# Eclectic-Sheep/sheeprl

Hardware: NVIDIA H100
Metric: Dreamer-V3 train-steps/sec (S, bs16 seq64 horizon15, 64x64x3 obs) (higher is better)
Workload: dtype f32

## Files before the change

### sheeprl_b200/csrc/gemm_tc.cu

```cuda
#include <cuda.h>
#include <cudaTypedefs.h>

#include <mutex>
#include <unordered_map>

#include "common.cuh"

namespace {

constexpr int BM = 128, BK = 32;
constexpr int NTHREADS = 384;
constexpr int NSPLIT_THREADS = 96;
constexpr int NCONS_WARPS = 8;
constexpr int PRODUCER_REGS = 56, CONSUMER_REGS = 224;
template <int BN> constexpr int stages_for() { return BN == 128 ? 3 : 5; }

__device__ __forceinline__ uint32_t smem_u32(const void* p) { return (uint32_t)__cvta_generic_to_shared(p); }

__device__ __forceinline__ void mbar_init(uint64_t* bar, uint32_t count) {
  asm volatile("mbarrier.init.shared::cta.b64 [%0], %1;" ::"r"(smem_u32(bar)), "r"(count) : "memory");
}
__device__ __forceinline__ void mbar_expect_tx(uint64_t* bar, uint32_t bytes) {
  asm volatile("mbarrier.arrive.expect_tx.shared::cta.b64 _, [%0], %1;" ::"r"(smem_u32(bar)), "r"(bytes) : "memory");
}
__device__ __forceinline__ void mbar_arrive(uint64_t* bar) {
  asm volatile("mbarrier.arrive.shared::cta.b64 _, [%0];" ::"r"(smem_u32(bar)) : "memory");
}
__device__ __forceinline__ bool mbar_try_wait(uint64_t* bar, uint32_t parity) {
  uint32_t ok;
  asm volatile(
      "{\n\t"
      ".reg .pred p;\n\t"
      "mbarrier.try_wait.parity.shared::cta.b64 p, [%1], %2;\n\t"
      "selp.u32 %0, 1, 0, p;\n\t"
      "}"
      : "=r"(ok)
      : "r"(smem_u32(bar)), "r"(parity)
      : "memory");
  return ok != 0;
}
__device__ __forceinline__ void mbar_wait(uint64_t* bar, uint32_t parity) {
  if (mbar_try_wait(bar, parity)) return;
  const long long t0 = clock64();
  while (!mbar_try_wait(bar, parity)) {
    if (clock64() - t0 > 2000000000LL) asm volatile("trap;");
  }
}
__device__ __forceinline__ bool elect_one() {
  uint32_t pred;
  asm volatile(
      "{\n\t"
      ".reg .pred p;\n\t"
      "elect.sync _|p, 0xffffffff;\n\t"
      "selp.u32 %0, 1, 0, p;\n\t"
      "}"
      : "=r"(pred));
  return pred != 0;
}
__device__ __forceinline__ void tma_load_2d(void* smem_dst, const CUtensorMap* map, uint64_t* bar, int c0, int c1) {
  asm volatile(
      "cp.async.bulk.tensor.2d.shared::cluster.global.mbarrier::complete_tx::bytes [%0], [%1, {%3, %4}], [%2];" ::"r"(
          smem_u32(smem_dst)),
      "l"(map), "r"(smem_u32(bar)), "r"(c0), "r"(c1)
      : "memory");
}
__device__ __forceinline__ void tma_load_4d(void* smem_dst, const CUtensorMap* map, uint64_t* bar, int c0, int c1, int c2,
                                            int c3) {
  asm volatile(
      "cp.async.bulk.tensor.4d.shared::cluster.global.mbarrier::complete_tx::bytes [%0], [%1, {%3, %4, %5, %6}], [%2];" ::"r"(
          smem_u32(smem_dst)),
      "l"(map), "r"(smem_u32(bar)), "r"(c0), "r"(c1), "r"(c2), "r"(c3)
      : "memory");
}

__device__ __forceinline__ void wgmma_tf32(float (&d)[32], const uint32_t (&a)[4], uint64_t desc_b, int scale_d) {
  asm volatile(
      "{\n\t.reg .pred p;\n\tsetp.ne.b32 p, %37, 0;\n\twgmma.mma_async.sync.aligned.m64n64k8.f32.tf32.tf32 {%0, %1, %2, %3, %4, %5, %6, %7, %8, %9, %10, %11, %12, %13, %14, %15, %16, %17, %18, %19, %20, %21, %22, %23, %24, %25, %26, %27, %28, %29, %30, %31}, {%32, %33, %34, %35}, %36, p, 1, 1;\n\t}"
      : "+f"(d[0]), "+f"(d[1]), "+f"(d[2]), "+f"(d[3]), "+f"(d[4]), "+f"(d[5]), "+f"(d[6]), "+f"(d[7]), "+f"(d[8]), "+f"(d[9]), "+f"(d[10]), "+f"(d[11]), "+f"(d[12]), "+f"(d[13]), "+f"(d[14]), "+f"(d[15]), "+f"(d[16]), "+f"(d[17]), "+f"(d[18]), "+f"(d[19]), "+f"(d[20]), "+f"(d[21]), "+f"(d[22]), "+f"(d[23]), "+f"(d[24]), "+f"(d[25]), "+f"(d[26]), "+f"(d[27]), "+f"(d[28]), "+f"(d[29]), "+f"(d[30]), "+f"(d[31])
      : "r"(a[0]), "r"(a[1]), "r"(a[2]), "r"(a[3]), "l"(desc_b), "r"(scale_d));
}
__device__ __forceinline__ void wgmma_tf32(float (&d)[64], const uint32_t (&a)[4], uint64_t desc_b, int scale_d) {
  asm volatile(
      "{\n\t.reg .pred p;\n\tsetp.ne.b32 p, %69, 0;\n\twgmma.mma_async.sync.aligned.m64n128k8.f32.tf32.tf32 {%0, %1, %2, %3, %4, %5, %6, %7, %8, %9, %10, %11, %12, %13, %14, %15, %16, %17, %18, %19, %20, %21, %22, %23, %24, %25, %26, %27, %28, %29, %30, %31, %32, %33, %34, %35, %36, %37, %38, %39, %40, %41, %42, %43, %44, %45, %46, %47, %48, %49, %50, %51, %52, %53, %54, %55, %56, %57, %58, %59, %60, %61, %62, %63}, {%64, %65, %66, %67}, %68, p, 1, 1;\n\t}"
      : "+f"(d[0]), "+f"(d[1]), "+f"(d[2]), "+f"(d[3]), "+f"(d[4]), "+f"(d[5]), "+f"(d[6]), "+f"(d[7]), "+f"(d[8]), "+f"(d[9]), "+f"(d[10]), "+f"(d[11]), "+f"(d[12]), "+f"(d[13]), "+f"(d[14]), "+f"(d[15]), "+f"(d[16]), "+f"(d[17]), "+f"(d[18]), "+f"(d[19]), "+f"(d[20]), "+f"(d[21]), "+f"(d[22]), "+f"(d[23]), "+f"(d[24]), "+f"(d[25]), "+f"(d[26]), "+f"(d[27]), "+f"(d[28]), "+f"(d[29]), "+f"(d[30]), "+f"(d[31]), "+f"(d[32]), "+f"(d[33]), "+f"(d[34]), "+f"(d[35]), "+f"(d[36]), "+f"(d[37]), "+f"(d[38]), "+f"(d[39]), "+f"(d[40]), "+f"(d[41]), "+f"(d[42]), "+f"(d[43]), "+f"(d[44]), "+f"(d[45]), "+f"(d[46]), "+f"(d[47]), "+f"(d[48]), "+f"(d[49]), "+f"(d[50]), "+f"(d[51]), "+f"(d[52]), "+f"(d[53]), "+f"(d[54]), "+f"(d[55]), "+f"(d[56]), "+f"(d[57]), "+f"(d[58]), "+f"(d[59]), "+f"(d[60]), "+f"(d[61]), "+f"(d[62]), "+f"(d[63])
      : "r"(a[0]), "r"(a[1]), "r"(a[2]), "r"(a[3]), "l"(desc_b), "r"(scale_d));
}
__device__ __forceinline__ void wgmma_fence() { asm volatile("wgmma.fence.sync.aligned;" ::: "memory"); }
__device__ __forceinline__ void wgmma_commit() { asm volatile("wgmma.commit_group.sync.aligned;" ::: "memory"); }
__device__ __forceinline__ void wgmma_wait_all() { asm volatile("wgmma.wait_group.sync.aligned 0;" ::: "memory"); }
template <int N>
__device__ __forceinline__ void fence_regs(float (&r)[N]) {
#pragma unroll
  for (int i = 0; i < N; ++i) asm volatile("" : "+f"(r[i])::"memory");
}
template <int N, int W>
__device__ __forceinline__ void fence_regs(uint32_t (&r)[N][W]) {
#pragma unroll
  for (int i = 0; i < N; ++i)
#pragma unroll
    for (int j = 0; j < W; ++j) asm volatile("" : "+r"(r[i][j])::"memory");
}

__device__ __forceinline__ uint64_t make_desc(uint32_t smem_addr) {
  uint64_t d = 0;
  d |= (uint64_t)((smem_addr & 0x3FFFF) >> 4);
  d |= (uint64_t)1 << 16;
  d |= (uint64_t)(1024 >> 4) << 32;
  d |= (uint64_t)1 << 62;
  return d;
}

__device__ __forceinline__ uint32_t kmajor_off(int r, int k) {
  return (uint32_t)(r * 128 + ((((k >> 2) ^ r) & 7) << 4) + (k & 3) * 4);
}
__device__ __forceinline__ uint32_t mnmajor_off(int r, int k) {
  return (uint32_t)((r >> 5) * 4096 + k * 128 + (((((r & 31) >> 2) ^ k) & 7) << 4) + (r & 3) * 4);
}

template <int BN>
struct Smem {
  static constexpr int STAGES = stages_for<BN>();
  float a[STAGES][BM * BK];
  float b[STAGES][BN * BK];
  float b_hi[STAGES][BN * BK];
  float b_lo[STAGES][BN * BK];
  uint64_t full[STAGES], split[STAGES], empty[STAGES];
};

constexpr int CH = 4;

constexpr int MODE_GEMM = 0, MODE_DOWN = 1, MODE_UP = 2;
constexpr int MODE_UP4 = 3;
constexpr int GROUP_M = 16;
struct TileGeo {
  int mode;
  int h, w, NB;
  int bw, bh, bn;
  int tiles_x, tiles_y;
  int chunks;
  int Cout;
  int ksplits;
  float* part;
  int mpad, ldw;
  int force_part;
  int passes;
  int a_mn, b_mn;
  int mtiles;
  int ntiles;
  int wg;
};

template <int BN, int PASSES>
__global__ void __launch_bounds__(NTHREADS, 1)
gemm_tc_kernel(const __grid_constant__ CUtensorMap mapA, const __grid_constant__ CUtensorMap mapB, float* __restrict__ C,
               const float* __restrict__ bias, int M, int N, int K, int ldc, int accumulate, const TileGeo geo) {
  constexpr int STAGES = Smem<BN>::STAGES;
  extern __shared__ __align__(1024) unsigned char smem_raw[];
  Smem<BN>& s = *reinterpret_cast<Smem<BN>*>((reinterpret_cast<uintptr_t>(smem_raw) + 1023) & ~(uintptr_t)1023);
  const int warp = threadIdx.x >> 5, lane = threadIdx.x & 31;
  const int mtiles = geo.mtiles * geo.ntiles, tstride = gridDim.y;
  auto tile_mn = [&](int id, int& tm, int& tn) {
    if (geo.ntiles == 1) { tm = id; tn = 0; return; }
    const int per = GROUP_M * geo.ntiles, grp = id / per, first = grp * GROUP_M;
    const int gsz = min(GROUP_M, geo.mtiles - first), r = id - grp * per;
    tn = r / gsz;
    tm = first + (r - tn * gsz);
  };
  int kb_base = 0, nkb = (K + BK - 1) / BK;
  if (geo.mode == MODE_GEMM && geo.ksplits > 1) {
    const int per = (nkb + geo.ksplits - 1) / geo.ksplits;
    kb_base = (int)blockIdx.z * per;
    nkb = min(per, nkb - kb_base);
  }
  const int py = (int)blockIdx.z >> 1, px = (int)blockIdx.z & 1;
  auto tile_origin = [&](int id, int& tx0, int& ty0, int& tn0) {
    tx0 = (id % geo.tiles_x) * geo.bw;
    ty0 = ((id / geo.tiles_x) % geo.tiles_y) * geo.bh;
    tn0 = (id / (geo.tiles_x * geo.tiles_y)) * geo.bn;
  };

  if (threadIdx.x == 0) {
    for (int i = 0; i < STAGES; ++i) {
      mbar_init(&s.full[i], 1);
      mbar_init(&s.split[i], NSPLIT_THREADS / 32);
      mbar_init(&s.empty[i], NCONS_WARPS);
    }
    asm volatile("fence.mbarrier_init.release.cluster;" ::: "memory");
  }
  __syncthreads();

  if (warp < 4) {
    asm volatile("setmaxnreg.dec.sync.aligned.u32 %0;" ::"n"(PRODUCER_REGS));
    if (warp == 0) {
      const bool leader = elect_one();
      int it = 0;
      for (int tile = blockIdx.y; tile < mtiles; tile += tstride) {
        int tm, tn;
        tile_mn(tile, tm, tn);
        const int m0 = tm * BM, n0 = tn * BN;
        int tx0 = 0, ty0 = 0, tn0 = 0;
        if (geo.mode != MODE_GEMM) tile_origin(tm, tx0, ty0, tn0);
        for (int kb = 0; kb < nkb; ++kb, ++it) {
          const int st = it % STAGES;
          if (it >= STAGES) mbar_wait(&s.empty[st], ((it / STAGES) - 1) & 1);
          if (leader) {
            mbar_expect_tx(&s.full[st], (uint32_t)((BM + BN) * BK * sizeof(float)));
            if (geo.mode == MODE_GEMM) {
              const int k0 = (kb_base + kb) * BK;
              if (geo.wg) {
                const int x0 = k0 % geo.w, y0 = (k0 / geo.w) % geo.h, i0 = k0 / (geo.w * geo.h);
                for (int j = 0; j < BM / 32; ++j) {
                  const int r0 = m0 + 32 * j, tap = r0 / geo.Cout, ch = r0 - tap * geo.Cout;
                  tma_load_4d(s.a[st] + j * 1024, &mapA, &s.full[st], ch, 2 * x0 - 1 + (tap & 3), 2 * y0 - 1 + (tap >> 2), i0);
                }
              } else if (!geo.a_mn) tma_load_2d(s.a[st], &mapA, &s.full[st], k0, m0);
              else
                for (int j = 0; j < BM / 32; ++j) tma_load_2d(s.a[st] + j * 1024, &mapA, &s.full[st], m0 + 32 * j, k0);
              if (!geo.b_mn) tma_load_2d(s.b[st], &mapB, &s.full[st], k0, n0);
              else
                for (int j = 0; j < BN / 32; ++j) tma_load_2d(s.b[st] + j * 1024, &mapB, &s.full[st], n0 + 32 * j, k0);
            } else {
              const int tap = kb / geo.chunks, ch = (kb - tap * geo.chunks) * BK;
              int x, y;
              if (geo.mode == MODE_DOWN)     { x = 2 * tx0 - 1 + (tap & 3); y = 2 * ty0 - 1 + (tap >> 2); }
              else if (geo.mode == MODE_UP4) { x = tx0 + (tap % 3) - 1;     y = ty0 + (tap / 3) - 1; }
              else                           { x = tx0 + px - (tap & 1);    y = ty0 + py - (tap >> 1); }
              tma_load_4d(s.a[st], &mapA, &s.full[st], ch, x, y, tn0);
              tma_load_2d(s.b[st], &mapB, &s.full[st], kb * BK, n0 + (geo.mode == MODE_UP ? (int)blockIdx.z * geo.Cout : 0));
            }
          }
          __syncwarp();
        }
      }
    } else {
      const int t = threadIdx.x - 32;
      int ntl = 0;
      for (int tile = blockIdx.y; tile < mtiles; tile += tstride) ++ntl;
      const int total_kb = ntl * nkb;
      const bool b_mn = geo.b_mn != 0;
      for (int kb = 0; kb < total_kb; ++kb) {
        const int st = kb % STAGES;
        mbar_wait(&s.full[st], (kb / STAGES) & 1);
        const char* raw = reinterpret_cast<const char*>(s.b[st]);
        char* bh = reinterpret_cast<char*>(s.b_hi[st]);
        char* bl = reinterpret_cast<char*>(s.b_lo[st]);
        for (int w = t; w < BN * BK / 4; w += NSPLIT_THREADS) {
          int n, kc;
          float4 v;
          if (!b_mn) {
            n = w >> 3; kc = w & 7;
            v = *reinterpret_cast<const float4*>(raw + kmajor_off(n, 4 * kc));
          } else {
            n = w % BN; kc = w / BN;
            v.x = *reinterpret_cast<const float*>(raw + mnmajor_off(n, 4 * kc));
            v.y = *reinterpret_cast<const float*>(raw + mnmajor_off(n, 4 * kc + 1));
            v.z = *reinterpret_cast<const float*>(raw + mnmajor_off(n, 4 * kc + 2));
            v.w = *reinterpret_cast<const float*>(raw + mnmajor_off(n, 4 * kc + 3));
          }
          float4 h;
          h.x = __uint_as_float(__float_as_uint(v.x) & 0xffffe000u);
          h.y = __uint_as_float(__float_as_uint(v.y) & 0xffffe000u);
          h.z = __uint_as_float(__float_as_uint(v.z) & 0xffffe000u);
          h.w = __uint_as_float(__float_as_uint(v.w) & 0xffffe000u);
          const uint32_t o = kmajor_off(n, 4 * kc);
          *reinterpret_cast<float4*>(bh + o) = h;
          if (PASSES == 3) *reinterpret_cast<float4*>(bl + o) = make_float4(v.x - h.x, v.y - h.y, v.z - h.z, v.w - h.w);
        }
        asm volatile("fence.proxy.async.shared::cta;" ::: "memory");
        __syncwarp();
        if (lane == 0) mbar_arrive(&s.split[st]);
      }
    }
  } else {
    asm volatile("setmaxnreg.inc.sync.aligned.u32 %0;" ::"n"(CONSUMER_REGS));
    constexpr int NACC = BN / 2;
    const int cw = (warp >> 2) - 1, wq = warp & 3, g = lane >> 2, tq = lane & 3;
    const int r0 = cw * 64 + wq * 16 + g;
    const bool a_mn_tile = geo.a_mn != 0;
    const uint64_t dbh_base = make_desc(smem_u32(s.b_hi[0])), dbl_base = make_desc(smem_u32(s.b_lo[0]));
    constexpr uint64_t STAGE_STEP = (uint64_t)(BN * BK * sizeof(float)) >> 4;
    int it = 0;
    for (int tile = blockIdx.y; tile < mtiles; tile += tstride) {
      int tm, tn;
      tile_mn(tile, tm, tn);
      const int m0 = tm * BM, n0 = tn * BN;
      int tx0 = 0, ty0 = 0, tn0 = 0;
      if (geo.mode != MODE_GEMM) tile_origin(tm, tx0, ty0, tn0);
      float acc[NACC], cacc[NACC];
#pragma unroll
      for (int j = 0; j < NACC; ++j) { acc[j] = 0.f; cacc[j] = 0.f; }
      for (int kb = 0; kb < nkb; ++kb, ++it) {
        const int st = it % STAGES;
        const uint32_t ph = (it / STAGES) & 1;
        mbar_wait(&s.full[st], ph);
        mbar_wait(&s.split[st], ph);
        const char* araw = reinterpret_cast<const char*>(s.a[st]);
        uint32_t ahi[4][4], alo[4][4];
#pragma unroll
        for (int ks = 0; ks < 4; ++ks)
#pragma unroll
          for (int e = 0; e < 4; ++e) {
            const int r = r0 + 8 * (e & 1), k = 8 * ks + tq + 4 * (e >> 1);
            const uint32_t x = *reinterpret_cast<const uint32_t*>(araw + (a_mn_tile ? mnmajor_off(r, k) : kmajor_off(r, k)));
            ahi[ks][e] = x & 0xffffe000u;
            if (PASSES == 3) alo[ks][e] = __float_as_uint(__uint_as_float(x) - __uint_as_float(x & 0xffffe000u));
          }
        const bool chunk_start = (kb % CH) == 0;
        const uint64_t dbh0 = dbh_base + (uint64_t)st * STAGE_STEP, dbl0 = dbl_base + (uint64_t)st * STAGE_STEP;
        fence_regs(cacc);
        fence_regs(ahi);
        if (PASSES == 3) fence_regs(alo);
        wgmma_fence();
#pragma unroll
        for (int ks = 0; ks < 4; ++ks) {
          const uint64_t ob = (uint64_t)ks * 2;
          const int keep = !(chunk_start && ks == 0);
          if (PASSES == 3) {
            wgmma_tf32(cacc, ahi[ks], dbl0 + ob, keep);
            wgmma_tf32(cacc, alo[ks], dbh0 + ob, 1);
            wgmma_tf32(cacc, ahi[ks], dbh0 + ob, 1);
          } else {
            wgmma_tf32(cacc, ahi[ks], dbh0 + ob, keep);
          }
        }
        wgmma_commit();
        wgmma_wait_all();
        fence_regs(cacc);
        fence_regs(ahi);
        if (PASSES == 3) fence_regs(alo);
        __syncwarp();
        if (lane == 0) mbar_arrive(&s.empty[st]);
        if ((kb % CH) == CH - 1 || kb == nkb - 1) {
#pragma unroll
          for (int j = 0; j < NACC; ++j) acc[j] += cacc[j];
        }
      }
#pragma unroll
      for (int hh = 0; hh < 2; ++hh) {
        const int r = r0 + 8 * hh;
        const int row = m0 + r;
        bool row_ok = row < M;
        size_t row_off = (size_t)row * ldc;
        int wi = 0, hi = 0, ni = 0;
        if (geo.mode != MODE_GEMM) {
          wi = r % geo.bw; hi = (r / geo.bw) % geo.bh; ni = r / (geo.bw * geo.bh);
          const int n = tn0 + ni, y = ty0 + hi, x = tx0 + wi;
          row_ok = n < geo.NB;
          if (geo.mode == MODE_DOWN) row_off = (((size_t)n * geo.h + y) * geo.w + x) * (size_t)ldc;
          else row_off = (((size_t)n * (2 * geo.h) + (2 * y + py)) * (2 * geo.w) + (2 * x + px)) * (size_t)ldc;
        }
        if (geo.mode == MODE_UP4) {
          if (!row_ok) continue;
          const size_t n = (size_t)(tn0 + ni);
          const int y = ty0 + hi, x = tx0 + wi;
#pragma unroll
          for (int j = 0; j < NACC / 4; ++j) {
            const int c = 8 * j + 2 * tq, p = c >> 5, ch = c & 31;
            float* dst = C + ((n * (2 * geo.h) + (2 * y + (p >> 1))) * (2 * geo.w) + (2 * x + (p & 1))) * (size_t)32 + ch;
            float2 o = make_float2(acc[4 * j + 2 * hh], acc[4 * j + 2 * hh + 1]);
            if (bias) { o.x += bias[ch]; o.y += bias[ch + 1]; }
            *reinterpret_cast<float2*>(dst) = o;
          }
          continue;
        }
        if (geo.mode == MODE_GEMM && (geo.ksplits > 1 || geo.force_part)) {
          float* prow = geo.part + ((size_t)blockIdx.z * geo.mpad + (size_t)row) * geo.ldw + n0;
#pragma unroll
          for (int j = 0; j < NACC / 4; ++j)
            *reinterpret_cast<float2*>(prow + 8 * j + 2 * tq) = make_float2(acc[4 * j + 2 * hh], acc[4 * j + 2 * hh + 1]);
          continue;
        }
        if (!row_ok) continue;
        float* crow = C + row_off;
#pragma unroll
        for (int j = 0; j < NACC / 4; ++j) {
          const int cb = n0 + 8 * j + 2 * tq;
          float v0 = acc[4 * j + 2 * hh], v1 = acc[4 * j + 2 * hh + 1];
          if (cb + 1 < N && ((reinterpret_cast<uintptr_t>(crow + cb) & 7) == 0)) {
            if (bias) { v0 += bias[cb]; v1 += bias[cb + 1]; }
            if (accumulate) { const float2 q = *reinterpret_cast<const float2*>(crow + cb); v0 += q.x; v1 += q.y; }
            *reinterpret_cast<float2*>(crow + cb) = make_float2(v0, v1);
          } else {
            if (cb < N) crow[cb] = v0 + (bias ? bias[cb] : 0.f) + (accumulate ? crow[cb] : 0.f);
            if (cb + 1 < N) crow[cb + 1] = v1 + (bias ? bias[cb + 1] : 0.f) + (accumulate ? crow[cb + 1] : 0.f);
          }
        }
      }
    }
  }
}

struct MapKey {
  const void* ptr; int rows, cols, ld, box_rows;
  bool operator==(const MapKey& o) const { return ptr == o.ptr && rows == o.rows && cols == o.cols && ld == o.ld && box_rows == o.box_rows; }
};
struct MapHash {
  size_t operator()(const MapKey& k) const {
    size_t h = std::hash<const void*>()(k.ptr);
    h ^= std::hash<long long>()(((long long)k.rows << 32) ^ k.cols) + 0x9e3779b97f4a7c15ull + (h << 6) + (h >> 2);
    h ^= std::hash<long long>()(((long long)k.ld << 8) ^ k.box_rows) + 0x9e3779b97f4a7c15ull + (h << 6) + (h >> 2);
    return h;
  }
};
std::unordered_map<MapKey, CUtensorMap, MapHash> g_maps;
std::mutex g_maps_mu;

typedef CUresult (*EncodeTiledFn)(CUtensorMap*, CUtensorMapDataType, cuuint32_t, void*, const cuuint64_t*, const cuuint64_t*,
                                  const cuuint32_t*, const cuuint32_t*, CUtensorMapInterleave, CUtensorMapSwizzle,
                                  CUtensorMapL2promotion, CUtensorMapFloatOOBfill);
EncodeTiledFn encode_tiled() {
  static EncodeTiledFn fn = nullptr;
  if (!fn) {
    void* p = nullptr;
    cudaDriverEntryPointQueryResult q;
    if (cudaGetDriverEntryPoint("cuTensorMapEncodeTiled", &p, cudaEnableDefault, &q) == cudaSuccess &&
        q == cudaDriverEntryPointSuccess)
      fn = reinterpret_cast<EncodeTiledFn>(p);
  }
  return fn;
// ... 103 lines not shown
  const int py = par >> 1, px = par & 1;
  const int ky = (1 - py) + 2 * (t >> 1), kx = (1 - px) + 2 * (t & 1);
  P[idx] = W[((long long)cs * Cb + cb) * 16 + ky * 4 + kx];
}

__global__ void conv_pack_up4_kernel(const float* __restrict__ W, float* __restrict__ P, int Cs, int Cb) {
  const long long idx = (long long)blockIdx.x * blockDim.x + threadIdx.x;
  if (idx >= 36LL * Cs * Cb) return;
  const int cs = (int)(idx % Cs);
  const int shift = (int)((idx / Cs) % 9);
  const int cb = (int)((idx / (9LL * Cs)) % Cb);
  const int par = (int)(idx / (9LL * Cs * Cb));
  const int py = par >> 1, px = par & 1, dy = shift / 3 - 1, dx = shift % 3 - 1;
  const int j = py - dy, i = px - dx;
  float v = 0.f;
  if (j >= 0 && j <= 1 && i >= 0 && i <= 1) v = W[((long long)cs * Cb + cb) * 16 + ((1 - py) + 2 * j) * 4 + (1 - px) + 2 * i];
  P[idx] = v;
}
static bool conv_up_merged(int Cb) { return Cb == 32; }

int g_passes = 3;

struct SplitWs {
  float* part = nullptr;
  size_t floats = 0;
};
SplitWs g_split[16];
std::mutex g_split_mu;

int split_workspace(size_t need_floats, cudaStream_t st, float** part) {
  int dev = 0;
  RL_CUDA(cudaGetDevice(&dev));
  RL_CHECK_ARG(dev < 16, "split-K workspace: device index out of range");
  std::lock_guard<std::mutex> lk(g_split_mu);
  SplitWs& w = g_split[dev];
  if (need_floats > w.floats) {
    cudaStreamCaptureStatus cs = cudaStreamCaptureStatusNone;
    RL_CUDA(cudaStreamIsCapturing(st, &cs));
    if (cs != cudaStreamCaptureStatusNone) {
      b200rl_set_error("split-K workspace must grow during stream capture: run the step once eagerly first");
      return B200RL_ERR_CUDA;
    }
    RL_CUDA(cudaDeviceSynchronize());
    if (w.part) RL_CUDA(cudaFree(w.part));
    const size_t n = need_floats + need_floats / 2 > (size_t)16 << 20 ? need_floats + need_floats / 2 : (size_t)16 << 20;
    RL_CUDA(cudaMalloc(&w.part, n * sizeof(float)));
    w.floats = n;
  }
  *part = w.part;
  return B200RL_OK;
}

__global__ void __launch_bounds__(256)
splitk_reduce_kernel(const float* __restrict__ part, float* __restrict__ C, const float* __restrict__ bias, int M, int N,
                     int ldc, int ks, int mpad, int ldw, int accumulate) {
  const int n4 = (N + 3) >> 2;
  const long long idx = (long long)blockIdx.x * blockDim.x + threadIdx.x;
  if (idx >= (long long)M * n4) return;
  const int m = (int)(idx / n4), n = (int)(idx - (long long)m * n4) * 4;
  const float* p = part + (size_t)m * ldw + n;
  float4 acc = make_float4(0.f, 0.f, 0.f, 0.f);
#pragma unroll 4
  for (int z = 0; z < ks; ++z) {
    const float4 v = __ldcg(reinterpret_cast<const float4*>(p + (size_t)z * mpad * ldw));
    acc.x += v.x; acc.y += v.y; acc.z += v.z; acc.w += v.w;
  }
  float* c = C + (size_t)m * ldc + n;
  const float o[4] = {acc.x, acc.y, acc.z, acc.w};
  if (n + 4 <= N && ((reinterpret_cast<uintptr_t>(c) & 15) == 0)) {
    float4 r = acc;
    if (bias) { r.x += bias[n]; r.y += bias[n + 1]; r.z += bias[n + 2]; r.w += bias[n + 3]; }
    if (accumulate) { const float4 q = *reinterpret_cast<const float4*>(c); r.x += q.x; r.y += q.y; r.z += q.z; r.w += q.w; }
    *reinterpret_cast<float4*>(c) = r;
  } else {
    for (int j = 0; j < 4 && n + j < N; ++j) {
      float r = o[j];
      if (bias) r += bias[n + j];
      if (accumulate) r += c[j];
      c[j] = r;
    }
  }
}

#define LAUNCH_GEMM_TC(BN_, PASSES_, grid_, st_, ...)                                                                \
  do {                                                                                                               \
    const size_t smem__ = sizeof(Smem<BN_>) + 1024;                                                                  \
    RL_CUDA(cudaFuncSetAttribute(gemm_tc_kernel<BN_, PASSES_>, cudaFuncAttributeMaxDynamicSharedMemorySize, (int)smem__)); \
    gemm_tc_kernel<BN_, PASSES_><<<grid_, NTHREADS, smem__, st_>>>(__VA_ARGS__);                                      \
  } while (0)
#define DISPATCH_GEMM_TC(BN_val, passes_val, grid_, st_, ...)                                  \
  do {                                                                                          \
    if ((BN_val) == 64) {                                                                       \
      if ((passes_val) == 3) LAUNCH_GEMM_TC(64, 3, grid_, st_, __VA_ARGS__);                    \
      else LAUNCH_GEMM_TC(64, 1, grid_, st_, __VA_ARGS__);                                      \
    } else {                                                                                    \
      if ((passes_val) == 3) LAUNCH_GEMM_TC(128, 3, grid_, st_, __VA_ARGS__);                   \
      else LAUNCH_GEMM_TC(128, 1, grid_, st_, __VA_ARGS__);                                     \
    }                                                                                           \
  } while (0)

int launch_conv(int mode, const float* img, const float* Wp, float* out, const float* bias, int NB, int h, int w, int Cin,
                int Cout, cudaStream_t st) {
  TileGeo g = {};
  g.mode = mode; g.h = h; g.w = w; g.NB = NB; g.chunks = Cin / BK; g.Cout = Cout; g.ksplits = 1;
  g.passes = g_passes;
  RL_CHECK_ARG(conv_tile(h, w, NB, &g.bw, &g.bh, &g.bn), "image grid not tileable by 128 pixels");
  g.tiles_x = w / g.bw; g.tiles_y = h / g.bh;
  if (mode == MODE_UP && conv_up_merged(Cout)) mode = g.mode = MODE_UP4;
  const int taps = mode == MODE_DOWN ? 16 : (mode == MODE_UP4 ? 9 : 4);
  const int K = taps * Cin;
  CUtensorMap ma, mb;
  if (mode == MODE_DOWN) { if (int rc = get_map4(img, Cin, 2 * w, 2 * h, NB, g.bw, g.bh, g.bn, 2, &ma)) return rc; }
  else                   { if (int rc = get_map4(img, Cin, w, h, NB, g.bw, g.bh, g.bn, 1, &ma)) return rc; }
  const int BN = (mode == MODE_UP4) ? 128 : ((Cout <= 64) ? 64 : 128);
  const int brows = (mode == MODE_UP || mode == MODE_UP4) ? 4 * Cout : Cout;
  if (int rc = get_map(Wp, brows, K, K, BN, &mb)) return rc;
  const int mtiles = g.tiles_x * g.tiles_y * (NB / g.bn);
  g.mtiles = mtiles;
  g.ntiles = (mode == MODE_UP4) ? 1 : (Cout + BN - 1) / BN;
  dim3 grid(1, 1, mode == MODE_UP ? 4 : 1);
  grid.y = persistent_grid_y(mtiles * g.ntiles, grid.z);
  const int M = NB * h * w;
  DISPATCH_GEMM_TC(BN, g.passes, grid, st, ma, mb, out, bias, M, Cout, K, Cout, 0, g);
  RL_CHECK_LAUNCH();
  return B200RL_OK;
}

}

extern "C" int b200rl_set_matmul_precision(int tf32_passes) {
  RL_CHECK_ARG(tf32_passes == 1 || tf32_passes == 3, "tf32_passes must be 3 (fp32-accurate 3xTF32) or 1 (single TF32 pass)");
  g_passes = tf32_passes;
  return B200RL_OK;
}
extern "C" int b200rl_get_matmul_precision(void) { return g_passes; }

extern "C" long long b200rl_conv_pack_floats(int mode_up, int Cs, int Cb) {
  return (mode_up && conv_up_merged(Cb) ? 36LL : 16LL) * Cs * Cb;
}
extern "C" int b200rl_conv_tc_supported(int mode_up, int NB, int h, int w, int Cs, int Cb) {
  int bw, bh, bn;
  if (!conv_tile(h, w, NB, &bw, &bh, &bn)) return 0;
  const int Cin = mode_up ? Cs : Cb, Cout = mode_up ? Cb : Cs;
  if (Cin % BK != 0 || Cout < 16 || Cout % 4 != 0) return 0;
  return 1;
}
extern "C" int b200rl_conv_pack(const float* W, float* Wpacked, int mode_up, int Cs, int Cb, cudaStream_t st) {
  RL_CHECK_ARG(W && Wpacked, "null pointer");
  const long long n = (long long)Cs * Cb * 16;
  if (mode_up && conv_up_merged(Cb)) conv_pack_up4_kernel<<<ceil_div(36LL * Cs * Cb, 256), 256, 0, st>>>(W, Wpacked, Cs, Cb);
  else if (mode_up) conv_pack_up_kernel<<<ceil_div(n, 256), 256, 0, st>>>(W, Wpacked, Cs, Cb);
  else conv_pack_down_kernel<<<ceil_div(n, 256), 256, 0, st>>>(W, Wpacked, Cs, Cb);
  RL_CHECK_LAUNCH();
  return B200RL_OK;
}
extern "C" int b200rl_conv_down_tc(const float* big, const float* Wpacked, float* small_, int NB, int h, int w, int Cs,
                                   int Cb, cudaStream_t st) {
  RL_CHECK_ARG(big && Wpacked && small_, "null pointer");
  RL_CHECK_ARG(b200rl_conv_tc_supported(0, NB, h, w, Cs, Cb), "shape not eligible for the tensor-core conv path");
  return launch_conv(MODE_DOWN, big, Wpacked, small_, nullptr, NB, h, w, Cb, Cs, st);
}
extern "C" int b200rl_conv_up_tc(const float* small_, const float* Wpacked, float* big, const float* bias, int NB, int h,
                                 int w, int Cs, int Cb, cudaStream_t st) {
  RL_CHECK_ARG(big && Wpacked && small_, "null pointer");
  RL_CHECK_ARG(b200rl_conv_tc_supported(1, NB, h, w, Cs, Cb), "shape not eligible for the tensor-core conv path");
  return launch_conv(MODE_UP, small_, Wpacked, big, bias, NB, h, w, Cs, Cb, st);
}

extern "C" int b200rl_gemm_tc_supported(const float* A, const float* B, int M, int N, int K, int lda, int ldb,
                                        int transA, int transB) {
  (void)transA; (void)transB;
  if (M < 32 || N < 48 || K < 32) return 0;
  if ((lda & 3) || (ldb & 3)) return 0;
  if ((reinterpret_cast<uintptr_t>(A) & 15) || (reinterpret_cast<uintptr_t>(B) & 15)) return 0;
  return 1;
}

namespace {
struct FusedTail { float* part; int ks, mpad, ldw; };

int gemm_tc_impl(const float* A, const float* B, float* C, const float* bias, int M, int N, int K, int lda,
                 int ldb, int ldc, int transA, int transB, int accumulate, cudaStream_t st, FusedTail* fused) {
  RL_CHECK_ARG(A && B && (C || fused), "null pointer");
  RL_CHECK_ARG(b200rl_gemm_tc_supported(A, B, M, N, K, lda, ldb, transA, transB), "shape not eligible for the tensor-core path");
  const int BN = (N <= 64) ? 64 : 128;
  CUtensorMap ma, mb;
  if (!transA) { if (int rc = get_map(A, M, K, lda, BM, &ma)) return rc; }
  else         { if (int rc = get_map(A, K, M, lda, 32, &ma)) return rc; }
  if (transB)  { if (int rc = get_map(B, N, K, ldb, BN, &mb)) return rc; }
  else         { if (int rc = get_map(B, K, N, ldb, 32, &mb)) return rc; }
  dim3 grid((N + BN - 1) / BN, (M + BM - 1) / BM);
  TileGeo g = {};
  g.mode = MODE_GEMM;
  g.a_mn = transA ? 1 : 0;
  g.b_mn = transB ? 0 : 1;
  g.ksplits = 1;
  g.passes = g_passes;
  const int tiles = grid.x * grid.y, nkb = (K + BK - 1) / BK;
  if (tiles < 2 * kNumSMs && nkb >= 8) {
    int best = 1;
    float best_t = 1e30f;
    const int max_sp = nkb / 4 < 32 ? nkb / 4 : 32;
    for (int sp = 1; sp <= (max_sp < 1 ? 1 : max_sp); ++sp) {
      const int per = (nkb + sp - 1) / sp, real = (nkb + per - 1) / per;
      const int waves = (tiles * real + kNumSMs - 1) / kNumSMs;
      const float t = waves * (per * 0.8f + 4.0f) + (real > 1 ? 3.0f + 0.3f * real : 0.0f);
      if (t < best_t - 1e-3f) { best_t = t; best = real; }
    }
    g.ksplits = best;
  }
  if (g.ksplits > 1 || fused) {
    grid.z = g.ksplits;
    g.mpad = (int)grid.y * BM;
    g.ldw = (int)grid.x * BN;
    if (int rc = split_workspace((size_t)g.ksplits * g.mpad * g.ldw, st, &g.part)) return rc;
    if (fused) { g.force_part = 1; *fused = FusedTail{g.part, g.ksplits, g.mpad, g.ldw}; }
  }
  g.mtiles = (int)grid.y;
  g.ntiles = (int)grid.x;
  grid.x = 1;
  grid.y = persistent_grid_y(g.mtiles * g.ntiles, grid.z);
  DISPATCH_GEMM_TC(BN, g.passes, grid, st, ma, mb, C, bias, M, N, K, ldc, accumulate, g);
  RL_CHECK_LAUNCH();
  if (g.ksplits > 1 && !fused) {
    splitk_reduce_kernel<<<ceil_div((long long)M * ((N + 3) / 4), 256), 256, 0, st>>>(g.part, C, bias, M, N, ldc, g.ksplits, g.mpad,
                                                                                      g.ldw, accumulate);
    RL_CHECK_LAUNCH();
  }
  return B200RL_OK;
}

template <int NV>
__global__ void __launch_bounds__(256)
splitk_ln_kernel(const float* __restrict__ part, int ks, int mpad, int ldw, int M, int N, const float* __restrict__ gamma,
                 const float* __restrict__ beta, float eps, int act, float* __restrict__ pre, long long ldpre,
                 float* __restrict__ ln_out, long long ldln, int mode, const float* __restrict__ h_prev, long long ldh,
                 float* __restrict__ h_out, long long ldho, float* __restrict__ h_out2, long long ldho2) {
  const int lane = threadIdx.x & 31;
  const long long row = ((long long)blockIdx.x * blockDim.x + threadIdx.x) >> 5;
  if (row >= M) return;
  const int n4 = N >> 2;
  float4 v[NV];
#pragma unroll
  for (int i = 0; i < NV; ++i) v[i] = make_float4(0.f, 0.f, 0.f, 0.f);
#pragma unroll 4
  for (int z = 0; z < ks; ++z) {
    const float4* p = reinterpret_cast<const float4*>(part + ((size_t)z * mpad + row) * ldw);
#pragma unroll
    for (int i = 0; i < NV; ++i) {
      const int c = lane + 32 * i;
      if (c < n4) { const float4 t = __ldcg(p + c); v[i].x += t.x; v[i].y += t.y; v[i].z += t.z; v[i].w += t.w; }
    }
  }
  float s = 0.f;
#pragma unroll
  for (int i = 0; i < NV; ++i) {
    const int c = lane + 32 * i;
    if (c < n4) {
      if (pre) reinterpret_cast<float4*>(pre + row * ldpre)[c] = v[i];
      s += (v[i].x + v[i].y) + (v[i].z + v[i].w);
    }
  }
  const float mu = warp_sum(s) / (float)N;
  float q = 0.f;
#pragma unroll
  for (int i = 0; i < NV; ++i) {
    const int c = lane + 32 * i;
    if (c < n4) {
      const float dx = v[i].x - mu, dy = v[i].y - mu, dz = v[i].z - mu, dw = v[i].w - mu;
      q += (dx * dx + dy * dy) + (dz * dz + dw * dw);
    }
  }
  const float rstd = rsqrtf(warp_sum(q) / (float)N + eps);
#pragma unroll
  for (int i = 0; i < NV; ++i) {
    const int c = lane + 32 * i;
    if (c < n4) {
      const float4 g = reinterpret_cast<const float4*>(gamma)[c], b = reinterpret_cast<const float4*>(beta)[c];
      v[i].x = (v[i].x - mu) * rstd * g.x + b.x; v[i].y = (v[i].y - mu) * rstd * g.y + b.y;
      v[i].z = (v[i].z - mu) * rstd * g.z + b.z; v[i].w = (v[i].w - mu) * rstd * g.w + b.w;
      if (mode == 0 && act == 1) {
        v[i].x = v[i].x / (1.f + expf(-v[i].x)); v[i].y = v[i].y / (1.f + expf(-v[i].y));
        v[i].z = v[i].z / (1.f + expf(-v[i].z)); v[i].w = v[i].w / (1.f + expf(-v[i].w));
      }
      if (ln_out) reinterpret_cast<float4*>(ln_out + row * ldln)[c] = v[i];
    }
  }
  if (mode == 1) {
    constexpr int NR = NV / 3;
#pragma unroll
    for (int i = 0; i < NR; ++i) {
      const int c = lane + 32 * i;
      const float4 hp = reinterpret_cast<const float4*>(h_prev + row * ldh)[c];
      const float4 gr = v[i], gc = v[i + NR], gu = v[i + 2 * NR];
      float4 h;
      auto gate = [](float r_, float c_, float u_, float hprev) {
        const float r = 1.f / (1.f + expf(-r_));
        const float cand = tanhf(r * c_);
        const float u = 1.f / (1.f + expf(-(u_ - 1.f)));
        return u * cand + (1.f - u) * hprev;
      };
      h.x = gate(gr.x, gc.x, gu.x, hp.x); h.y = gate(gr.y, gc.y, gu.y, hp.y);
      h.z = gate(gr.z, gc.z, gu.z, hp.z); h.w = gate(gr.w, gc.w, gu.w, hp.w);
      reinterpret_cast<float4*>(h_out + row * ldho)[c] = h;
      if (h_out2) reinterpret_cast<float4*>(h_out2 + row * ldho2)[c] = h;
    }
  }
}
}

extern "C" int b200rl_gemm_tc(const float* A, const float* B, float* C, const float* bias, int M, int N, int K, int lda,
                              int ldb, int ldc, int transA, int transB, int accumulate, cudaStream_t st) {
  return gemm_tc_impl(A, B, C, bias, M, N, K, lda, ldb, ldc, transA, transB, accumulate, st, nullptr);
}

extern "C" int b200rl_gemm_ln_supported(const float* A, const float* B, int M, int N, int K, int lda, int ldb, int mode) {
  if (!b200rl_gemm_tc_supported(A, B, M, N, K, lda, ldb, 0, 1)) return 0;
  if (N % 4 || N > 1536) return 0;
  if (mode == 1 && (N % 384 != 0)) return 0;
  return 1;
}

extern "C" int b200rl_gemm_ln(const float* A, const float* W, int M, int N, int K, int lda, int ldw_, const float* gamma,
                              const float* beta, float eps, int act, float* pre, long long ldpre, float* out, long long ldout,
                              int mode, const float* h_prev, long long ldh, float* h_out, long long ldho, float* h_out2,
                              long long ldho2, cudaStream_t st) {
  RL_CHECK_ARG(A && W && gamma && beta, "null pointer");
  RL_CHECK_ARG(b200rl_gemm_ln_supported(A, W, M, N, K, lda, ldw_, mode), "shape not eligible for the fused product + LayerNorm");
  RL_CHECK_ARG(mode == 0 ? out != nullptr : (h_prev && h_out), "missing output");
  RL_CHECK_ARG(((reinterpret_cast<uintptr_t>(gamma) | reinterpret_cast<uintptr_t>(beta) | reinterpret_cast<uintptr_t>(pre) |
                 reinterpret_cast<uintptr_t>(out) | reinterpret_cast<uintptr_t>(h_prev) | reinterpret_cast<uintptr_t>(h_out) |
                 reinterpret_cast<uintptr_t>(h_out2)) & 15) == 0 &&
                   ((ldpre | ldout | ldh | ldho | ldho2) & 3) == 0,
               "fused product + LayerNorm needs 16-byte aligned rows");
  FusedTail ft;
  if (int rc = gemm_tc_impl(A, W, nullptr, nullptr, M, N, K, lda, ldw_, N, 0, 1, 0, st, &ft)) return rc;
  const int blocks = ceil_div((long long)M * 32, 256);
#define LAUNCH_SPLITK_LN(NV_)                                                                                              \
  splitk_ln_kernel<NV_><<<blocks, 256, 0, st>>>(ft.part, ft.ks, ft.mpad, ft.ldw, M, N, gamma, beta, eps, act, pre, ldpre, out, \
                                                ldout, mode, h_prev, ldh, h_out, ldho, h_out2, ldho2)
  if (mode == 1) {
    if (N == 384) LAUNCH_SPLITK_LN(3); else if (N == 768) LAUNCH_SPLITK_LN(6); else if (N == 1152) LAUNCH_SPLITK_LN(9);
    else LAUNCH_SPLITK_LN(12);
  } else if (N <= 128) LAUNCH_SPLITK_LN(1);
  else if (N <= 256) LAUNCH_SPLITK_LN(2);
  else if (N <= 512) LAUNCH_SPLITK_LN(4);
  else if (N <= 1024) LAUNCH_SPLITK_LN(8);
  else LAUNCH_SPLITK_LN(12);
#undef LAUNCH_SPLITK_LN
  RL_CHECK_LAUNCH();
  return B200RL_OK;
}

extern "C" int b200rl_conv_wgrad_mn_supported(int NB, int h, int w, int Cs, int Cb) {
  if (w <= 0 || h <= 0 || (w & (w - 1)) || (h & (h - 1))) return 0;
  const long long P = (long long)NB * h * w;
  if (Cb % 32 || Cs < 48 || Cs % 4 || P % 32 || P < 1024 || P > 2000000000LL) return 0;
  const int bw = w < 32 ? w : 32, bh = (32 / bw) < h ? (32 / bw) : h, bn = 32 / (bw * bh);
  return (bw * bh * bn == 32) && (NB % bn == 0);
}

extern "C" int b200rl_conv_wgrad_mn(const float* small_, const float* big, float* G, int NB, int h, int w, int Cs, int Cb,
                                    cudaStream_t st) {
  RL_CHECK_ARG(small_ && big && G, "null pointer");
  RL_CHECK_ARG(b200rl_conv_wgrad_mn_supported(NB, h, w, Cs, Cb), "shape not eligible for the in-place wgrad path");
  const int P = NB * h * w, M = 16 * Cb, N = Cs;
  TileGeo g = {};
  g.mode = MODE_GEMM; g.a_mn = 1; g.b_mn = 1; g.wg = 1; g.passes = g_passes;
  g.h = h; g.w = w; g.NB = NB; g.Cout = Cb;
  g.bw = w < 32 ? w : 32; g.bh = (32 / g.bw) < h ? (32 / g.bw) : h; g.bn = 32 / (g.bw * g.bh);
  CUtensorMap ma, mb;
  if (int rc = get_map4(big, Cb, 2 * w, 2 * h, NB, g.bw, g.bh, g.bn, 2, &ma)) return rc;
  if (int rc = get_map(small_, P, Cs, Cs, 32, &mb)) return rc;
  const int BN = (N <= 64) ? 64 : 128;
  dim3 grid((N + BN - 1) / BN, M / BM);
  const int tiles = grid.x * grid.y, nkb = P / BK;
  int sp = (2 * kNumSMs + tiles - 1) / tiles;
  if (sp > nkb / 8) sp = nkb / 8;
  if (sp < 1) sp = 1;
  const int per = (nkb + sp - 1) / sp;
  g.ksplits = (nkb + per - 1) / per;
  grid.z = g.ksplits;
  g.mtiles = (int)grid.y;
  g.ntiles = (int)grid.x;
  if (g.ksplits > 1) {
    g.mpad = (int)grid.y * BM;
    g.ldw = (int)grid.x * BN;
    if (int rc = split_workspace((size_t)g.ksplits * g.mpad * g.ldw, st, &g.part)) return rc;
  }
  grid.x = 1;
  grid.y = (unsigned)(g.mtiles * g.ntiles);
  DISPATCH_GEMM_TC(BN, g.passes, grid, st, ma, mb, G, nullptr, M, N, P, N, 0, g);
  RL_CHECK_LAUNCH();
  if (g.ksplits > 1) {
    splitk_reduce_kernel<<<ceil_div((long long)M * ((N + 3) / 4), 256), 256, 0, st>>>(g.part, G, nullptr, M, N, N, g.ksplits, g.mpad,
                                                                                      g.ldw, 0);
    RL_CHECK_LAUNCH();
  }
  return B200RL_OK;
}
```

Baseline: 50.33.

## Keep one wgmma group in flight, specialize K-major B, and size stages to smem

Adds a KMAJOR_B template parameter so K-major B tiles are fed to wgmma straight from the TMA buffer, with no hi-copy by the split warps. When passes is 1 those warps skip splitting entirely. The consumer loop now double-buffers A fragments and waits with wait_group 1 instead of 0, loading the next stage's fragments while the current MMA runs. Stage count is derived from the 227KB shared-memory budget, and the wgrad split-k heuristic rounds down instead of up. This adds template variants and more complex release ordering, and the timeout handling changes from trap-in-loop to a flag.

After: 51.48 (median of 6 runs). 2.3% higher.

```diff
diff --git a/sheeprl_b200/csrc/gemm_tc.cu b/sheeprl_b200/csrc/gemm_tc.cu
--- a/sheeprl_b200/csrc/gemm_tc.cu
+++ b/sheeprl_b200/csrc/gemm_tc.cu
@@ -13,7 +13,6 @@
 constexpr int NSPLIT_THREADS = 96;
 constexpr int NCONS_WARPS = 8;
 constexpr int PRODUCER_REGS = 56, CONSUMER_REGS = 224;
-template <int BN> constexpr int stages_for() { return BN == 128 ? 3 : 5; }
 
 __device__ __forceinline__ uint32_t smem_u32(const void* p) { return (uint32_t)__cvta_generic_to_shared(p); }
 
@@ -46,6 +45,11 @@
     if (clock64() - t0 > 2000000000LL) asm volatile("trap;");
   }
 }
+__device__ __forceinline__ void mbar_wait_flag(uint64_t* bar, uint32_t parity, bool& timed_out) {
+  if (mbar_try_wait(bar, parity)) return;
+  const long long t0 = clock64();
+  while (!timed_out && !mbar_try_wait(bar, parity)) timed_out = clock64() - t0 > 2000000000LL;
+}
 __device__ __forceinline__ bool elect_one() {
   uint32_t pred;
   asm volatile(
@@ -87,7 +91,8 @@
 }
 __device__ __forceinline__ void wgmma_fence() { asm volatile("wgmma.fence.sync.aligned;" ::: "memory"); }
 __device__ __forceinline__ void wgmma_commit() { asm volatile("wgmma.commit_group.sync.aligned;" ::: "memory"); }
-__device__ __forceinline__ void wgmma_wait_all() { asm volatile("wgmma.wait_group.sync.aligned 0;" ::: "memory"); }
+template <int N>
+__device__ __forceinline__ void wgmma_wait() { asm volatile("wgmma.wait_group.sync.aligned %0;" ::"n"(N) : "memory"); }
 template <int N>
 __device__ __forceinline__ void fence_regs(float (&r)[N]) {
 #pragma unroll
@@ -117,14 +122,17 @@
   return (uint32_t)((r >> 5) * 4096 + k * 128 + (((((r & 31) >> 2) ^ k) & 7) << 4) + (r & 3) * 4);
 }
 
-template <int BN>
+template <int BN, bool KMAJOR_B>
 struct Smem {
-  static constexpr int STAGES = stages_for<BN>();
+  static constexpr int NSPLITB = KMAJOR_B ? 1 : 2;
+  static constexpr int STAGE_BYTES = (BM + (1 + NSPLITB) * BN) * BK * 4 + 3 * 8;
+  static constexpr int STAGES = (227 * 1024 - 1024) / STAGE_BYTES;
   float a[STAGES][BM * BK];
   float b[STAGES][BN * BK];
-  float b_hi[STAGES][BN * BK];
-  float b_lo[STAGES][BN * BK];
+  float bs[NSPLITB][STAGES][BN * BK];
   uint64_t full[STAGES], split[STAGES], empty[STAGES];
+  __device__ float* b_hi(int st) { return KMAJOR_B ? b[st] : bs[0][st]; }
+  __device__ float* b_lo(int st) { return bs[NSPLITB - 1][st]; }
 };
 
 constexpr int CH = 4;
@@ -150,13 +158,15 @@
   int wg;
 };
 
-template <int BN, int PASSES>
+template <int BN, int PASSES, bool KMAJOR_B>
 __global__ void __launch_bounds__(NTHREADS, 1)
 gemm_tc_kernel(const __grid_constant__ CUtensorMap mapA, const __grid_constant__ CUtensorMap mapB, float* __restrict__ C,
                const float* __restrict__ bias, int M, int N, int K, int ldc, int accumulate, const TileGeo geo) {
-  constexpr int STAGES = Smem<BN>::STAGES;
+  using Sm = Smem<BN, KMAJOR_B>;
+  constexpr int STAGES = Sm::STAGES;
+  constexpr bool SPLIT_B = PASSES == 3 || !KMAJOR_B;
   extern __shared__ __align__(1024) unsigned char smem_raw[];
-  Smem<BN>& s = *reinterpret_cast<Smem<BN>*>((reinterpret_cast<uintptr_t>(smem_raw) + 1023) & ~(uintptr_t)1023);
+  Sm& s = *reinterpret_cast<Sm*>((reinterpret_cast<uintptr_t>(smem_raw) + 1023) & ~(uintptr_t)1023);
   const int warp = threadIdx.x >> 5, lane = threadIdx.x & 31;
   const int mtiles = geo.mtiles * geo.ntiles, tstride = gridDim.y;
   auto tile_mn = [&](int id, int& tm, int& tn) {
@@ -216,7 +226,7 @@
               } else if (!geo.a_mn) tma_load_2d(s.a[st], &mapA, &s.full[st], k0, m0);
               else
                 for (int j = 0; j < BM / 32; ++j) tma_load_2d(s.a[st] + j * 1024, &mapA, &s.full[st], m0 + 32 * j, k0);
-              if (!geo.b_mn) tma_load_2d(s.b[st], &mapB, &s.full[st], k0, n0);
+              if (KMAJOR_B) tma_load_2d(s.b[st], &mapB, &s.full[st], k0, n0);
               else
                 for (int j = 0; j < BN / 32; ++j) tma_load_2d(s.b[st] + j * 1024, &mapB, &s.full[st], n0 + 32 * j, k0);
             } else {
@@ -232,22 +242,21 @@
           __syncwarp();
         }
       }
-    } else {
+    } else if (SPLIT_B) {
       const int t = threadIdx.x - 32;
       int ntl = 0;
       for (int tile = blockIdx.y; tile < mtiles; tile += tstride) ++ntl;
       const int total_kb = ntl * nkb;
-      const bool b_mn = geo.b_mn != 0;
       for (int kb = 0; kb < total_kb; ++kb) {
         const int st = kb % STAGES;
         mbar_wait(&s.full[st], (kb / STAGES) & 1);
         const char* raw = reinterpret_cast<const char*>(s.b[st]);
-        char* bh = reinterpret_cast<char*>(s.b_hi[st]);
-        char* bl = reinterpret_cast<char*>(s.b_lo[st]);
+        char* bh = reinterpret_cast<char*>(s.b_hi(st));
+        char* bl = reinterpret_cast<char*>(s.b_lo(st));
         for (int w = t; w < BN * BK / 4; w += NSPLIT_THREADS) {
           int n, kc;
           float4 v;
-          if (!b_mn) {
+          if (KMAJOR_B) {
             n = w >> 3; kc = w & 7;
             v = *reinterpret_cast<const float4*>(raw + kmajor_off(n, 4 * kc));
           } else {
@@ -263,7 +272,7 @@
           h.z = __uint_as_float(__float_as_uint(v.z) & 0xffffe000u);
           h.w = __uint_as_float(__float_as_uint(v.w) & 0xffffe000u);
           const uint32_t o = kmajor_off(n, 4 * kc);
-          *reinterpret_cast<float4*>(bh + o) = h;
+          if (!KMAJOR_B) *reinterpret_cast<float4*>(bh + o) = h;
           if (PASSES == 3) *reinterpret_cast<float4*>(bl + o) = make_float4(v.x - h.x, v.y - h.y, v.z - h.z, v.w - h.w);
         }
         asm volatile("fence.proxy.async.shared::cta;" ::: "memory");
@@ -277,8 +286,31 @@
     const int cw = (warp >> 2) - 1, wq = warp & 3, g = lane >> 2, tq = lane & 3;
     const int r0 = cw * 64 + wq * 16 + g;
     const bool a_mn_tile = geo.a_mn != 0;
-    const uint64_t dbh_base = make_desc(smem_u32(s.b_hi[0])), dbl_base = make_desc(smem_u32(s.b_lo[0]));
+    const uint64_t dbh_base = make_desc(smem_u32(s.b_hi(0))), dbl_base = make_desc(smem_u32(s.b_lo(0)));
     constexpr uint64_t STAGE_STEP = (uint64_t)(BN * BK * sizeof(float)) >> 4;
+    constexpr bool INFLIGHT = KMAJOR_B;
+    auto release = [&](int i) {
+      __syncwarp();
+      if (lane == 0) mbar_arrive(&s.empty[i % STAGES]);
+    };
+    bool timed_out = false;
+    auto load_frag = [&](int i, uint32_t (&hi)[4][4], uint32_t (&lo)[4][4]) {
+      const int st = i % STAGES;
+      const uint32_t ph = (i / STAGES) & 1;
+      mbar_wait_flag(&s.full[st], ph, timed_out);
+      if (SPLIT_B) mbar_wait_flag(&s.split[st], ph, timed_out);
+      const char* araw = reinterpret_cast<const char*>(s.a[st]);
+#pragma unroll
+      for (int ks = 0; ks < 4; ++ks)
+#pragma unroll
+        for (int e = 0; e < 4; ++e) {
+          const int r = r0 + 8 * (e & 1), k = 8 * ks + tq + 4 * (e >> 1);
+          const uint32_t x = *reinterpret_cast<const uint32_t*>(araw + (a_mn_tile ? mnmajor_off(r, k) : kmajor_off(r, k)));
+          hi[ks][e] = x & 0xffffe000u;
+          if (PASSES == 3) lo[ks][e] = __float_as_uint(__uint_as_float(x) - __uint_as_float(x & 0xffffe000u));
+        }
+    };
+    uint32_t ahi0[4][4] = {}, alo0[4][4] = {}, ahi1[4][4] = {}, alo1[4][4] = {};
     int it = 0;
     for (int tile = blockIdx.y; tile < mtiles; tile += tstride) {
       int tm, tn;
@@ -289,52 +321,59 @@
       float acc[NACC], cacc[NACC];
 #pragma unroll
       for (int j = 0; j < NACC; ++j) { acc[j] = 0.f; cacc[j] = 0.f; }
-      for (int kb = 0; kb < nkb; ++kb, ++it) {
-        const int st = it % STAGES;
-        const uint32_t ph = (it / STAGES) & 1;
-        mbar_wait(&s.full[st], ph);
-        mbar_wait(&s.split[st], ph);
-        const char* araw = reinterpret_cast<const char*>(s.a[st]);
-        uint32_t ahi[4][4], alo[4][4];
-#pragma unroll
-        for (int ks = 0; ks < 4; ++ks)
-#pragma unroll
-          for (int e = 0; e < 4; ++e) {
-            const int r = r0 + 8 * (e & 1), k = 8 * ks + tq + 4 * (e >> 1);
-            const uint32_t x = *reinterpret_cast<const uint32_t*>(araw + (a_mn_tile ? mnmajor_off(r, k) : kmajor_off(r, k)));
-            ahi[ks][e] = x & 0xffffe000u;
-            if (PASSES == 3) alo[ks][e] = __float_as_uint(__uint_as_float(x) - __uint_as_float(x & 0xffffe000u));
-          }
-        const bool chunk_start = (kb % CH) == 0;
+      auto step = [&](int kb, uint32_t (&hi)[4][4], uint32_t (&lo)[4][4], uint32_t (&nhi)[4][4], uint32_t (&nlo)[4][4]) {
+        const int i = it + kb, st = i % STAGES;
+        const bool chunk_start = (kb % CH) == 0, chunk_end = (kb % CH) == CH - 1 || kb == nkb - 1;
         const uint64_t dbh0 = dbh_base + (uint64_t)st * STAGE_STEP, dbl0 = dbl_base + (uint64_t)st * STAGE_STEP;
         fence_regs(cacc);
-        fence_regs(ahi);
-        if (PASSES == 3) fence_regs(alo);
+        fence_regs(hi);
+        if (PASSES == 3) fence_regs(lo);
         wgmma_fence();
 #pragma unroll
         for (int ks = 0; ks < 4; ++ks) {
           const uint64_t ob = (uint64_t)ks * 2;
           const int keep = !(chunk_start && ks == 0);
           if (PASSES == 3) {
-            wgmma_tf32(cacc, ahi[ks], dbl0 + ob, keep);
-            wgmma_tf32(cacc, alo[ks], dbh0 + ob, 1);
-            wgmma_tf32(cacc, ahi[ks], dbh0 + ob, 1);
+            wgmma_tf32(cacc, hi[ks], dbl0 + ob, keep);
+            wgmma_tf32(cacc, lo[ks], dbh0 + ob, 1);
+            wgmma_tf32(cacc, hi[ks], dbh0 + ob, 1);
           } else {
-            wgmma_tf32(cacc, ahi[ks], dbh0 + ob, keep);
+            wgmma_tf32(cacc, hi[ks], dbh0 + ob, keep);
           }
         }
         wgmma_commit();
-        wgmma_wait_all();
-        fence_regs(cacc);
-        fence_regs(ahi);
-        if (PASSES == 3) fence_regs(alo);
-        __syncwarp();
-        if (lane == 0) mbar_arrive(&s.empty[st]);
-        if ((kb % CH) == CH - 1 || kb == nkb - 1) {
+        if (INFLIGHT) {
+          wgmma_wait<1>();
+          fence_regs(nhi);
+          if (PASSES == 3) fence_regs(nlo);
+          if (!chunk_start) release(i - 1);
+        } else {
+          wgmma_wait<0>();
+          fence_regs(cacc);
+          fence_regs(hi);
+          if (PASSES == 3) fence_regs(lo);
+          release(i);
+        }
+        if (kb + 1 < nkb) load_frag(i + 1, nhi, nlo);
+        if (chunk_end) {
+          if (INFLIGHT) {
+            wgmma_wait<0>();
+            fence_regs(cacc);
+            fence_regs(hi);
+            if (PASSES == 3) fence_regs(lo);
+            release(i);
+          }
 #pragma unroll
           for (int j = 0; j < NACC; ++j) acc[j] += cacc[j];
         }
+      };
+      load_frag(it, ahi0, alo0);
+      for (int kb = 0; kb < nkb; kb += 2) {
+        step(kb, ahi0, alo0, ahi1, alo1);
+        if (kb + 1 < nkb) step(kb + 1, ahi1, alo1, ahi0, alo0);
       }
+      it += nkb;
+      if (timed_out) asm volatile("trap;");
 #pragma unroll
       for (int hh = 0; hh < 2; ++hh) {
         const int r = r0 + 8 * hh;
@@ -604,20 +643,27 @@
   }
 }
 
-#define LAUNCH_GEMM_TC(BN_, PASSES_, grid_, st_, ...)                                                                \
+#define LAUNCH_GEMM_TC(BN_, PASSES_, KMAJOR_B_, grid_, st_, ...)                                                     \
   do {                                                                                                               \
-    const size_t smem__ = sizeof(Smem<BN_>) + 1024;                                                                  \
-    RL_CUDA(cudaFuncSetAttribute(gemm_tc_kernel<BN_, PASSES_>, cudaFuncAttributeMaxDynamicSharedMemorySize, (int)smem__)); \
-    gemm_tc_kernel<BN_, PASSES_><<<grid_, NTHREADS, smem__, st_>>>(__VA_ARGS__);                                      \
+    constexpr size_t smem__ = sizeof(Smem<BN_, KMAJOR_B_>) + 1024;                                                   \
+    static_assert(smem__ <= 227 * 1024, "operand stages exceed the shared memory of an SM");                        \
+    RL_CUDA(cudaFuncSetAttribute(gemm_tc_kernel<BN_, PASSES_, KMAJOR_B_>, cudaFuncAttributeMaxDynamicSharedMemorySize, \
+                                 (int)smem__));                                                                      \
+    gemm_tc_kernel<BN_, PASSES_, KMAJOR_B_><<<grid_, NTHREADS, smem__, st_>>>(__VA_ARGS__);                           \
   } while (0)
-#define DISPATCH_GEMM_TC(BN_val, passes_val, grid_, st_, ...)                                  \
+#define DISPATCH_GEMM_TC_B(BN_, KMAJOR_B_, passes_val, grid_, st_, ...)                        \
+  do {                                                                                          \
+    if ((passes_val) == 3) LAUNCH_GEMM_TC(BN_, 3, KMAJOR_B_, grid_, st_, __VA_ARGS__);          \
+    else LAUNCH_GEMM_TC(BN_, 1, KMAJOR_B_, grid_, st_, __VA_ARGS__);                            \
+  } while (0)
+#define DISPATCH_GEMM_TC(BN_val, b_mn_val, passes_val, grid_, st_, ...)                        \
   do {                                                                                          \
     if ((BN_val) == 64) {                                                                       \
-      if ((passes_val) == 3) LAUNCH_GEMM_TC(64, 3, grid_, st_, __VA_ARGS__);                    \
-      else LAUNCH_GEMM_TC(64, 1, grid_, st_, __VA_ARGS__);                                      \
+      if (b_mn_val) DISPATCH_GEMM_TC_B(64, false, passes_val, grid_, st_, __VA_ARGS__);         \
+      else DISPATCH_GEMM_TC_B(64, true, passes_val, grid_, st_, __VA_ARGS__);                   \
     } else {                                                                                    \
-      if ((passes_val) == 3) LAUNCH_GEMM_TC(128, 3, grid_, st_, __VA_ARGS__);                   \
-      else LAUNCH_GEMM_TC(128, 1, grid_, st_, __VA_ARGS__);                                     \
+      if (b_mn_val) DISPATCH_GEMM_TC_B(128, false, passes_val, grid_, st_, __VA_ARGS__);        \
+      else DISPATCH_GEMM_TC_B(128, true, passes_val, grid_, st_, __VA_ARGS__);                  \
     }                                                                                           \
   } while (0)
 
@@ -643,7 +689,7 @@
   dim3 grid(1, 1, mode == MODE_UP ? 4 : 1);
   grid.y = persistent_grid_y(mtiles * g.ntiles, grid.z);
   const int M = NB * h * w;
-  DISPATCH_GEMM_TC(BN, g.passes, grid, st, ma, mb, out, bias, M, Cout, K, Cout, 0, g);
+  DISPATCH_GEMM_TC(BN, g.b_mn, g.passes, grid, st, ma, mb, out, bias, M, Cout, K, Cout, 0, g);
   RL_CHECK_LAUNCH();
   return B200RL_OK;
 }
@@ -742,7 +788,7 @@
   g.ntiles = (int)grid.x;
   grid.x = 1;
   grid.y = persistent_grid_y(g.mtiles * g.ntiles, grid.z);
-  DISPATCH_GEMM_TC(BN, g.passes, grid, st, ma, mb, C, bias, M, N, K, ldc, accumulate, g);
+  DISPATCH_GEMM_TC(BN, g.b_mn, g.passes, grid, st, ma, mb, C, bias, M, N, K, ldc, accumulate, g);
   RL_CHECK_LAUNCH();
   if (g.ksplits > 1 && !fused) {
     splitk_reduce_kernel<<<ceil_div((long long)M * ((N + 3) / 4), 256), 256, 0, st>>>(g.part, C, bias, M, N, ldc, g.ksplits, g.mpad,
@@ -897,7 +943,7 @@
   const int BN = (N <= 64) ? 64 : 128;
   dim3 grid((N + BN - 1) / BN, M / BM);
   const int tiles = grid.x * grid.y, nkb = P / BK;
-  int sp = (2 * kNumSMs + tiles - 1) / tiles;
+  int sp = 2 * kNumSMs / tiles;
   if (sp > nkb / 8) sp = nkb / 8;
   if (sp < 1) sp = 1;
   const int per = (nkb + sp - 1) / sp;
@@ -912,7 +958,7 @@
   }
   grid.x = 1;
   grid.y = (unsigned)(g.mtiles * g.ntiles);
-  DISPATCH_GEMM_TC(BN, g.passes, grid, st, ma, mb, G, nullptr, M, N, P, N, 0, g);
+  DISPATCH_GEMM_TC(BN, g.b_mn, g.passes, grid, st, ma, mb, G, nullptr, M, N, P, N, 0, g);
   RL_CHECK_LAUNCH();
   if (g.ksplits > 1) {
     splitk_reduce_kernel<<<ceil_div((long long)M * ((N + 3) / 4), 256), 256, 0, st>>>(g.part, G, nullptr, M, N, N, g.ksplits, g.mpad,
```
